# ru1ven/KeypointFusion

Measured on AMD Instinct MI355X. Metric: RGB-D img/sec fwd (B=64, 256x256), higher is better.
Workload: dtype f32; 1 GPU; KPFusion-convnext-tiny, depth+RGB UNet backbones forward, B=64/GPU 256x256 f32 (BASELINE configs[1]); batch_per_gpu=64, global_batch=64, input=256x256, parallelism=dp1 (batch shards, no collective)

## Files before the change

### include/kpf.h

```cpp
#ifndef KPF_H
#define KPF_H

#ifdef __cplusplus
extern "C" {
#endif

#define KPF_OK 0
#define KPF_EINVAL (-1)
#define KPF_ELAUNCH (-2)

#define KPF_DT_F32 0
#define KPF_DT_BF16 1
#define KPF_DT_F16 2
#define KPF_DT_F32_MMA_BF16 8
#define KPF_DT_F32_MMA_F16 9

#define KPF_ACT_RELU 1u
#define KPF_ACT_GELU 2u
#define KPF_RES_ADD 4u
#define KPF_RES_GAMMA 8u
#define KPF_RELU_AFTER_RES 16u
#define KPF_ACT_LEAKY 64u
#define KPF_IN_SPLIT 128u
#define KPF_W_SPLIT 512u
// ... 437 lines not shown
int kpf_geom_gate_forward(const float* pix_xyz, const float* joint_xyz, float* gam, int B, int J, int P, void* stream);
int kpf_geom_gate_backward(const float* pix_xyz, const float* joint_xyz, const float* dgam, float* djoint, int B, int J, int P, void* stream);

int kpf_geom_gate_uvd_forward(const float* pix_xyz, const float* joint_uvd, const float* par16, float* gam, int B, int J, int P, float half_size, float flip,
                              void* stream);
int kpf_geom_gate_uvd_backward(const float* pix_xyz, const float* joint_uvd, const float* par16, const float* dgam, float* djoint_uvd, int B, int J, int P,
                               float half_size, float flip, void* stream);

int kpf_prep_crop_u16(const unsigned char* rgb, const unsigned short* depth, const double* bbox, const double* cam, const double* cube, int B, int Hs, int Ws,
                      int x0, int y0, int H, int W, int S, float* img, float* img_rgb, float* center, float* M, float* cube_out, float* cam_para, double* com,
                      int* bounds, double* M64, void* stream);

int kpf_prep_pcl_sample(const float* img, const float* center, const double* M64, const double* cube, const double* cam, const long long* seed, int B, int S,
                        int n, float* pcl, int* pcl_index, int* pcl_count, float* cand_pts, void* stream);

int kpf_prep_uncrop_f32(const float* joints, const float* center, const float* M, const float* cube, const float* cam, int B, int J, float* crop_px,
                        float* frame_px, void* stream);

int kpf_prep_set_stamps(void* stamps64 );

int kpf_eval_errors_f32(const float* const* stages, int S, const float* gt, const float* cube, const int* score_index, int B, int J, int Jsel, float* err,
                        void* stream);

int kpf_eval_accumulate(const float* err, const unsigned char* valid, const double* thresholds, int S, int B, int Jsel, int T, long long* n_samples,
                        long long* n_batches, double* sum_err, double* sum_pa, double* sum_batch_mean, double* sum_batch_pa_mean, long long* pck,
                        long long* pck_pa, void* stream);

int kpf_prep_crop_u16_indexed(const unsigned char* rgb, const unsigned short* depth, const int* frame_index, int F, const double* bbox, const double* cam,
                              const double* cube, int B, int Hs, int Ws, int x0, int y0, int H, int W, int S, float* img, float* img_rgb, float* center, float* M,
                              float* cube_out, float* cam_para, double* com, int* bounds, double* M64, void* stream);

int kpf_track_step_f32(const float* joints, const float* center, const float* M, const float* cube, const float* cam_para, const int* pcl_count, int B, int J,
                       int frame_w, int frame_h, float expansion, long long seed_stride, double* bbox, long long* seed, int* lost, float* crop_px,
                       float* frame_px, float* cam_mm, double* bbox_used, int* status, void* stream);

int kpf_prep_annot_u16(const unsigned char* rgb, const unsigned short* depth, const int* frame_index, int F, const float* joints_mm, const float* cam32,
                       const float* center_xyz, const unsigned char* mirror, const double* cube, int B, int J, int Hs, int Ws, int x0, int y0, int H, int W, int S,
                       float* img, float* img_rgb, float* center, float* M, float* cube_out, float* cam_para, double* com, int* bounds, double* M64, float* joint,
                       float* joint_img, double* cam64, void* stream);

int kpf_prep_uncrop_mirror_f32(const float* joints, const float* center, const float* M, const float* cube, const float* cam, const unsigned char* mirror,
                               int frame_w, int B, int J, float* crop_px, float* frame_px, void* stream);

int kpf_prep_augment_u16(const unsigned char* rgb, const unsigned short* depth, const int* frame_index, int F, const float* joints_mm, const float* cam32,
                         const float* center_xyz, const unsigned char* mirror, const double* cube, const int* mode, const double* off, const double* sc,
                         const double* rot, const double* rot_cs, const double* color, int B, int J, int Hs, int Ws, int x0, int y0, int H, int W, int S,
                         float* img, float* img_rgb, float* center, float* M, float* cube_out, float* cam_para, double* com, int* bounds, double* M64,
                         float* joint, float* joint_img, double* cam64, double* cube64, int* aug_status, void* stream);

int kpf_prep_aug_draw(long long* seed, int B, double sigma_com, double sigma_sc, double rot_range, double color_factor, long long seed_stride, int* mode,
                      double* off, double* sc, double* rot, double* rot_cs, double* color, void* stream);

int kpf_conv_num_tile_cfgs(void);

const char* kpf_last_error(void);
#define KPF_ABI_VERSION 31
int kpf_abi_version(void);

#ifdef __cplusplus
}
#endif
#endif
```

### keypointfusion_amd/csrc/kpf_conv.hip

```cpp
#include "kpf_common.h"
#include <stdlib.h>
#include <type_traits>

namespace {

struct ConvArgs {
  const float* in;
  const float* w;
  const float* bias;
  const float* ps;
  const float* pt;
  const float* gamma;
  const float* res;
  float* out;
  int M, N, K, Kp;
  int IH, IW, Cin, in_ld, in_coff;
  int OH, OW, ohow, KH, KW, sh, sw, ph, pw;
  int out_ld, out_coff, res_ld, res_coff;
  const float* zero;
  float w_unscale;
  unsigned flags;
  int tilesN, nblk;
  int vec;
  int dbg;
  int st_policy;
  int skew;
  int groups, g_in, g_out;
  long g_w;
};

__device__ __forceinline__ ConvArgs kpf_group_args(const ConvArgs& a0) {
  ConvArgs a = a0;
  const int g = blockIdx.y;
  a.in_coff += g * a.g_in;
  a.out_coff += g * a.g_out;
  a.res_coff += g * a.g_out;
  a.w += (long)g * a.g_w;
  if (a.bias) a.bias += g * a.g_out;
  return a;
}

__device__ __forceinline__ float gelu_erf(float x) {
  const float z = fabsf(x) * 0.70710678118654752440f;
  const float t = __builtin_amdgcn_rcpf(fmaf(0.3275911f, z, 1.0f));
  float p = fmaf(1.061405429f, t, -1.453152027f);
  p = fmaf(p, t, 1.421413741f);
  p = fmaf(p, t, -0.284496736f);
  p = fmaf(p, t, 0.254829592f);
  const float e = __builtin_amdgcn_exp2f(-1.4426950408889634f * z * z);
  const float q = 0.5f * x * (p * t) * e;
  return fmaxf(x, 0.f) - fabsf(q);
}

// ... 149 lines not shown
      if (WHOLE || RPP * p + 8 * wave < BN)
        __builtin_amdgcn_global_load_lds((gbl_void_t*)(pb[p] + kt * BK), (lds_void_t*)(Bs + (RPP * p + 8 * wave) * BK), 16, 0, 0);
  };

  const f32x4 zero4 = {0.f, 0.f, 0.f, 0.f};
  f32x4 acc[TN][TM];
#pragma unroll
  for (int i = 0; i < TN; ++i)
#pragma unroll
    for (int j = 0; j < TM; ++j) acc[i][j] = zero4;

  const int nk = a.Kp / BK;
  const int fr = lane & 15;
  const int fg = lane >> 4;
  const int rsw = (fr >> 1) & 7;

  constexpr int EPW = H16 ? 2 : 1;
  float* pro_s = lds + NS * TILE;
  float* pro_t = pro_s + a.Kp * EPW;
  if (NS <= 2) {
    stage(0, 0);
  } else {
#pragma unroll
    for (int t = 0; t < NS - 1; ++t)
      if (t < nk) stage(t, t);
  }
  if (HAS_PRO) {
    for (int i = tid; i < a.Kp * EPW; i += 64 * NW) {
      pro_s[i] = i < a.Cin * EPW ? a.ps[i] : 0.f;
      pro_t[i] = i < a.Cin * EPW ? a.pt[i] : 0.f;
    }
  }
  if (NS <= 2) __syncthreads();

  KPF_STAMP(1);
  if constexpr (ARITH == ARITH_F32 && NS == 2) {
    auto read_frags = [&](int buf, int s16, f32x4(&xf)[TM], f32x4(&wf)[TN]) {
      const float* xrow = lds + buf * TILE + (wm * TM * 16 + fr) * BK;
      const float* wrow = lds + buf * TILE + BMR * BK + (wn * TN * 16 + fr) * BK;
      const int sc = (((4 * s16 + fg) ^ rsw) << 2);
#pragma unroll
      for (int j = 0; j < TM; ++j) xf[j] = *reinterpret_cast<const f32x4*>(xrow + j * 16 * BK + sc);
#pragma unroll
      for (int i = 0; i < TN; ++i) wf[i] = *reinterpret_cast<const f32x4*>(wrow + i * 16 * BK + sc);
    };
    auto prologue = [&](int kt, int s16, f32x4(&xf)[TM]) {
      if constexpr (HAS_PRO) {
        const int kk = kt * BK + 16 * s16 + 4 * fg;
        const f32x4 sp = *reinterpret_cast<const f32x4*>(pro_s + kk);
        const f32x4 tp = *reinterpret_cast<const f32x4*>(pro_t + kk);
#pragma unroll
        for (int j = 0; j < TM; ++j)
#pragma unroll
          for (int e = 0; e < 4; ++e) xf[j][e] = fmaxf(fmaf(xf[j][e], sp[e], tp[e]), 0.f);
      }
    };
    auto mma = [&](int e, const f32x4(&xf)[TM], const f32x4(&wf)[TN]) {
#pragma unroll
      for (int i = 0; i < TN; ++i)
#pragma unroll
        for (int j = 0; j < TM; ++j) acc[i][j] = __builtin_amdgcn_mfma_f32_16x16x4f32(wf[i][e], xf[j][e], acc[i][j], 0, 0, 0);
    };
    f32x4 xa[TM], wa[TN], xb[TM], wb[TN];
    read_frags(0, 0, xa, wa);
    if (nk > 1) stage(1, 1);
    for (int kt = 0; kt + 1 < nk; ++kt) {
      const int cur = kt & 1;
      read_frags(cur, 1, xb, wb);
      prologue(kt, 0, xa);
#pragma unroll
      for (int e = 0; e < 4; ++e) mma(e, xa, wa);
      prologue(kt, 1, xb);
#pragma unroll
      for (int e = 0; e < 3; ++e) mma(e, xb, wb);
      __builtin_amdgcn_sched_barrier(0);
      asm volatile("s_waitcnt vmcnt(0) lgkmcnt(0)" ::: "memory");
      __builtin_amdgcn_s_barrier();
      __builtin_amdgcn_sched_barrier(0);
      read_frags(cur ^ 1, 0, xa, wa);
      stage(kt + 2 < nk ? kt + 2 : nk - 1, cur);
      mma(3, xb, wb);
      __builtin_amdgcn_sched_group_barrier(0x100, TM + TN, 0);
#pragma unroll
      for (int q = 0; q < AP + BP; ++q) {
        __builtin_amdgcn_sched_group_barrier(0x008, (TM * TN) / (AP + BP) > 0 ? (TM * TN) / (AP + BP) : 1, 0);
        __builtin_amdgcn_sched_group_barrier(0x020, 1, 0);
      }
    }
    {
      const int kt = nk - 1, cur = kt & 1;
      read_frags(cur, 1, xb, wb);
      prologue(kt, 0, xa);
#pragma unroll
      for (int e = 0; e < 4; ++e) mma(e, xa, wa);
      prologue(kt, 1, xb);
#pragma unroll
      for (int e = 0; e < 4; ++e) mma(e, xb, wb);
    }
    asm volatile("s_waitcnt vmcnt(0)" ::: "memory");
  } else
  if constexpr (NS > 2 && ARITH == ARITH_SPLIT && !HAS_PRO) {
    const int ch = ((fg ^ rsw) << 2), cl = (((4 + fg) ^ rsw) << 2);
    auto read_frags = [&](int buf, f16x8(&xh)[TM], f16x8(&xl)[TM], f16x8(&wh)[TN], f16x8(&wl)[TN]) {
      const float* xrow = lds + buf * TILE + (wm * TM * 16 + fr) * BK;
      const float* wrow = lds + buf * TILE + BMR * BK + (wn * TN * 16 + fr) * BK;
#pragma unroll
      for (int j = 0; j < TM; ++j) {
// ... 137 lines not shown
          tp1 = *reinterpret_cast<const f32x4*>(pro_t + kk + 4);
        }
#pragma unroll
        for (int j = 0; j < TM; ++j) {
          f32x4 u0 = *reinterpret_cast<const f32x4*>(xrow + j * 16 * BK + c0);
          f32x4 u1 = *reinterpret_cast<const f32x4*>(xrow + j * 16 * BK + c1);
          if (HAS_PRO) {
#pragma unroll
            for (int e = 0; e < 4; ++e) {
              u0[e] = fmaxf(fmaf(u0[e], sp0[e], tp0[e]), 0.f);
              u1[e] = fmaxf(fmaf(u1[e], sp1[e], tp1[e]), 0.f);
            }
          }
#pragma unroll
          for (int e = 0; e < 4; ++e) {
            const float v0 = __builtin_amdgcn_fmed3f(u0[e], -65504.0f, 65504.0f), v1 = __builtin_amdgcn_fmed3f(u1[e], -65504.0f, 65504.0f);
            const _Float16 h0 = (_Float16)v0, h1 = (_Float16)v1;
            xh[j][e] = h0;
            xh[j][4 + e] = h1;
            xl[j][e] = (_Float16)(v0 - (float)h0);
            xl[j][4 + e] = (_Float16)(v1 - (float)h1);
          }
        }
      }
#pragma unroll
      for (int i = 0; i < TN; ++i) {
        wh[i] = *reinterpret_cast<const f16x8*>(wrow + i * 16 * BK + ch);
        wl[i] = *reinterpret_cast<const f16x8*>(wrow + i * 16 * BK + cl);
      }
#pragma unroll
      for (int i = 0; i < TN; ++i)
#pragma unroll
        for (int j = 0; j < TM; ++j) {
          acc[i][j] = __builtin_amdgcn_mfma_f32_16x16x32_f16(wl[i], xh[j], acc[i][j], 0, 0, 0);
          acc[i][j] = __builtin_amdgcn_mfma_f32_16x16x32_f16(wh[i], xl[j], acc[i][j], 0, 0, 0);
          acc[i][j] = __builtin_amdgcn_mfma_f32_16x16x32_f16(wh[i], xh[j], acc[i][j], 0, 0, 0);
        }
    } else {
#pragma unroll
      for (int s = 0; s < BK / 16; ++s) {
        const int sc = (((4 * s + fg) ^ rsw) << 2);
        f32x4 xf[TM], wf[TN];
#pragma unroll
        for (int j = 0; j < TM; ++j) xf[j] = *reinterpret_cast<const f32x4*>(xrow + j * 16 * BK + sc);
#pragma unroll
        for (int i = 0; i < TN; ++i) wf[i] = *reinterpret_cast<const f32x4*>(wrow + i * 16 * BK + sc);
        if (HAS_PRO) {
          const int kk = kt * BK + 16 * s + 4 * fg;
          const f32x4 sp = *reinterpret_cast<const f32x4*>(pro_s + kk);
          const f32x4 tp = *reinterpret_cast<const f32x4*>(pro_t + kk);
#pragma unroll
          for (int j = 0; j < TM; ++j)
#pragma unroll
            for (int e = 0; e < 4; ++e) xf[j][e] = fmaxf(fmaf(xf[j][e], sp[e], tp[e]), 0.f);
        }
        if constexpr (ARITH == ARITH_R_BF16 || ARITH == ARITH_R_F16) {
          typedef short r16x4 __attribute__((ext_vector_type(4)));
          r16x4 wh[TN], xh[TM];
#pragma unroll
          for (int i = 0; i < TN; ++i) {
            if constexpr (ARITH == ARITH_R_BF16) wh[i] = __builtin_bit_cast(r16x4, bf16x4{(bf16_t)wf[i][0], (bf16_t)wf[i][1], (bf16_t)wf[i][2], (bf16_t)wf[i][3]});
            else wh[i] = __builtin_bit_cast(r16x4, f16x4{(f16_t)wf[i][0], (f16_t)wf[i][1], (f16_t)wf[i][2], (f16_t)wf[i][3]});
          }
#pragma unroll
          for (int j = 0; j < TM; ++j) {
            if constexpr (ARITH == ARITH_R_BF16) xh[j] = __builtin_bit_cast(r16x4, bf16x4{(bf16_t)xf[j][0], (bf16_t)xf[j][1], (bf16_t)xf[j][2], (bf16_t)xf[j][3]});
            else xh[j] = __builtin_bit_cast(r16x4, f16x4{(f16_t)xf[j][0], (f16_t)xf[j][1], (f16_t)xf[j][2], (f16_t)xf[j][3]});
          }
#pragma unroll
          for (int i = 0; i < TN; ++i)
#pragma unroll
            for (int j = 0; j < TM; ++j) {
              if constexpr (ARITH == ARITH_R_BF16) acc[i][j] = __builtin_amdgcn_mfma_f32_16x16x16bf16_1k(wh[i], xh[j], acc[i][j], 0, 0, 0);
              else acc[i][j] = __builtin_amdgcn_mfma_f32_16x16x16f16(__builtin_bit_cast(f16x4, wh[i]), __builtin_bit_cast(f16x4, xh[j]), acc[i][j], 0, 0, 0);
            }
        } else {
#pragma unroll
          for (int e = 0; e < 4; ++e)
#pragma unroll
            for (int i = 0; i < TN; ++i)
#pragma unroll
              for (int j = 0; j < TM; ++j)
                acc[i][j] = __builtin_amdgcn_mfma_f32_16x16x4f32(wf[i][e], xf[j][e], acc[i][j], 0, 0, 0);
        }
      }
    }
    if (NS == 2) __syncthreads();
    if (NS == 1 && kt + 1 < nk) {
      __syncthreads();
      stage(kt + 1, 0);
      __syncthreads();
    }
  }

  KPF_STAMP(2);
  const unsigned fl = a.flags;
  const bool interior = (m0 + BM <= a.M) && (n0 + BN <= a.N) && a.vec && !(fl & KPF_OUT_NCHW);
  if (interior) {
    f32x4 bvv[TN], gvv[TN];
#pragma unroll
    for (int i = 0; i < TN; ++i) {
      const int n = n0 + (wn * TN + i) * 16 + fg * 4;
      bvv[i] = a.bias ? *reinterpret_cast<const f32x4*>(a.bias + n) : zero4;
      gvv[i] = (EPI == EPI_RES && (fl & KPF_RES_GAMMA)) ? *reinterpret_cast<const f32x4*>(a.gamma + n) : zero4;
    }
    constexpr bool HAS_RES = EPI == EPI_RES || EPI == EPI_GGRAD;
    constexpr bool STAGED = H16 && !HAS_RES && TN == 4;
    constexpr int RS = TN * 16 + 8;
    TH* stg = reinterpret_cast<TH*>(lds) + wave * (TM * 16) * RS;
    if constexpr (STAGED) __syncthreads();
    f32x4 rvv[HAS_RES ? TM : 1][TN];
    if (HAS_RES) {
#pragma unroll
      for (int j = 0; j < TM; ++j) {
        const long m = m0 + (wm * TM + j) * 16 + fr;
#pragma unroll
        for (int i = 0; i < TN; ++i) {
          const long o = m * a.res_ld + a.res_coff + n0 + (wn * TN + i) * 16 + fg * 4;
          if constexpr (H16) rvv[j][i] = kpf_ld4(reinterpret_cast<const TH*>(a.res) + o);
          else rvv[j][i] = *reinterpret_cast<const f32x4*>(a.res + o);
        }
      }
    }
#pragma unroll
    for (int j = 0; j < TM; ++j) {
      const long m = m0 + (wm * TM + j) * 16 + fr;
#pragma unroll
      for (int i = 0; i < TN; ++i) {
        const int n = n0 + (wn * TN + i) * 16 + fg * 4;
        const f32x4 bv = bvv[i], gv = gvv[i];
        f32x4 v = acc[i][j];
        if (SPLIT) {
#pragma unroll
          for (int e = 0; e < 4; ++e) v[e] *= a.w_unscale;
        }
        if (EPI == EPI_RES) {
#pragma unroll
          for (int e = 0; e < 4; ++e) {
            float y = v[e] + bv[e];
            if (fl & KPF_RES_GAMMA) y *= gv[e];
            y += rvv[HAS_RES ? j : 0][i][e];
            if (fl & KPF_RELU_AFTER_RES) y = fmaxf(y, 0.f);
            v[e] = y;
          }
        } else if (EPI == EPI_GGRAD) {
#pragma unroll
          for (int e = 0; e < 4; ++e) v[e] = (v[e] + bv[e]) * gelu_grad_erf(rvv[HAS_RES ? j : 0][i][e]);
        } else if (EPI == EPI_GELU) {
#pragma unroll
          for (int e = 0; e < 4; ++e) v[e] = gelu_of<ARITH>(v[e] + bv[e]);
        } else if (EPI == EPI_GELU2) {
          f32x4 z;
#pragma unroll
          for (int e = 0; e < 4; ++e) z[e] = v[e] + bv[e];
          if constexpr (H16) kpf_st4(reinterpret_cast<TH*>(const_cast<float*>(a.res)) + m * a.res_ld + a.res_coff + n, z);
          else STORE4(const_cast<float*>(a.res) + m * a.res_ld + a.res_coff + n, z);
#pragma unroll
          for (int e = 0; e < 4; ++e) {
            if constexpr (H16) z[e] = (float)(TH)z[e];
            v[e] = gelu_exact_erf(z[e]);
          }
        } else {
#pragma unroll
          for (int e = 0; e < 4; ++e) {
            const float y = v[e] + bv[e];
            v[e] = (fl & KPF_ACT_RELU) ? fmaxf(y, 0.f) : y;
          }
          if (fl & KPF_ACT_LEAKY) {
#pragma unroll
            for (int e = 0; e < 4; ++e) v[e] = fmaxf(v[e], 0.01f * v[e]);
          }
        }
        if constexpr (STAGED)
          kpf_st4(stg + (j * 16 + fr) * RS + i * 16 + fg * 4, v);
        else if constexpr (H16)
          kpf_st4(reinterpret_cast<TH*>(a.out) + m * a.out_ld + a.out_coff + n, v);
        else if (fl & KPF_OUT_SPLIT)
          kpf_store_split4(a.out + m * a.out_ld + a.out_coff, n, v);
        else if (a.st_policy == 2)
          asm volatile("global_store_dwordx4 %0, %1, off nt" ::"v"(a.out + m * a.out_ld + a.out_coff + n), "v"(v) : "memory");
        else
          STORE4(a.out + m * a.out_ld + a.out_coff + n, v);
      }
    }
    if constexpr (STAGED) {
      __syncthreads();
      TH* ob = reinterpret_cast<TH*>(a.out) + (long)(m0 + wm * TM * 16) * a.out_ld + a.out_coff + n0 + wn * TN * 16;
      const int prow = lane >> 3, pch = (lane & 7) * 8;
#pragma unroll
      for (int r = 0; r < TM * 2; ++r) {
        const int px = r * 8 + prow;
        const f32x4 q = *reinterpret_cast<const f32x4*>(stg + px * RS + pch);
        *reinterpret_cast<f32x4*>(ob + (long)px * a.out_ld + pch) = q;
      }
    }
    KPF_STAMP(3);
    return;
  }
  if constexpr (EPI == EPI_LIN) {
    if ((fl & KPF_OUT_NCHW) && a.ohow % BM == 0 && m0 + BM <= a.M && !(fl & KPF_OUT_SPLIT)) {
      constexpr int RS = BM + 4;
      static_assert(WN * 16 * RS <= NS * TILE, "the transpose staging fits the K buffers");
      const int b = m0 / a.ohow, pix0 = m0 - b * a.ohow;
#pragma unroll
      for (int i = 0; i < TN; ++i) {
        __syncthreads();
        const int nq = n0 + (wn * TN + i) * 16 + fg * 4;
        float bq[4];
#pragma unroll
        for (int e = 0; e < 4; ++e) bq[e] = (a.bias && nq + e < a.N) ? a.bias[nq + e] : 0.f;
#pragma unroll
        for (int j = 0; j < TM; ++j) {
          const int ml = (wm * TM + j) * 16 + fr;
#pragma unroll
          for (int e = 0; e < 4; ++e) {
            float y = (SPLIT ? acc[i][j][e] * a.w_unscale : acc[i][j][e]) + bq[e];
            if (fl & KPF_ACT_RELU) y = fmaxf(y, 0.f);
            if (fl & KPF_ACT_LEAKY) y = fmaxf(y, 0.01f * y);
            lds[(wn * 16 + fg * 4 + e) * RS + ml] = y;
          }
// ... 776 lines not shown
  KPF_REQUIRE(!(fl & KPF_RES_GELU_GRAD) || ((fl & KPF_RES_ADD) && !(fl & (KPF_RES_GAMMA | KPF_RELU_AFTER_RES | KPF_OUT_NCHW))), "kpf_conv2d_f32: RES_GELU_GRAD goes with RES_ADD alone");
  KPF_REQUIRE(!(fl & KPF_ACT_GELU_SAVE) || ((fl & KPF_ACT_GELU) && !(fl & (KPF_RES_ADD | KPF_OUT_NCHW)) && res && kpf_aligned16(res) && d->res_coff >= 0 && d->res_coff + d->N <= d->res_ld),
              "kpf_conv2d_f32: ACT_GELU_SAVE goes with ACT_GELU and a second output buffer in the res slot (res_ld / res_coff describe it)");
  KPF_REQUIRE((long)d->B * d->OH * d->OW < (1l << 31) && (long)d->B * d->IH * d->IW < (1l << 31), "kpf_conv2d_f32: too many pixels");

  ConvArgs a;
  a.in = in; a.w = w; a.bias = bias; a.ps = pro_scale; a.pt = pro_shift; a.gamma = gamma; a.res = res; a.out = out;
  a.M = d->B * d->OH * d->OW; a.N = d->N; a.K = d->KH * d->KW * d->Cin; a.Kp = d->Kp;
  a.IH = d->IH; a.IW = d->IW; a.Cin = d->Cin; a.in_ld = d->in_ld; a.in_coff = d->in_coff;
  a.OH = d->OH; a.OW = d->OW; a.ohow = d->OH * d->OW; a.KH = d->KH; a.KW = d->KW;
  a.sh = d->sh; a.sw = d->sw; a.ph = d->ph; a.pw = d->pw;
  a.out_ld = d->out_ld; a.out_coff = d->out_coff; a.res_ld = d->res_ld; a.res_coff = d->res_coff;
  {
    static const float* zero_of_dev[64] = {nullptr};
    int dev = 0;
    if (hipGetDevice(&dev) != hipSuccess || dev < 0 || dev >= 64) dev = 0;
    if (!zero_of_dev[dev]) {
      void* p = nullptr;
      if (hipGetSymbolAddress(&p, HIP_SYMBOL(kpf_zero16)) != hipSuccess || !p) {
        kpf_set_error("kpf_conv2d_f32: cannot resolve the zero page");
        return KPF_ELAUNCH;
      }
      zero_of_dev[dev] = static_cast<const float*>(p);
    }
    a.zero = zero_of_dev[dev];
  }
  a.flags = fl; a.tilesN = 0; a.nblk = 0; a.dbg = 0; a.skew = 0; a.st_policy = 0;
  {
    static const int st_mb = []() { const char* e = getenv("KPF_F32_ST_MB"); return e ? atoi(e) : 0; }();
    if (st_mb > 0 && (long)d->B * d->OH * d->OW * d->N * 4 >= (long)st_mb * 1000000) a.st_policy = 2;
  }
  a.w_unscale = (fl & (KPF_IN_SPLIT | KPF_W_SPLIT)) ? d->w_unscale : 1.0f;
  if (fl & (KPF_IN_SPLIT | KPF_W_SPLIT))
    KPF_REQUIRE(d->w_unscale > 0.f && d->Cin % 32 == 0 && d->in_coff % 4 == 0, "kpf_conv2d_f32: split operands need w_unscale > 0 and Cin %% 32 == 0 (Cin=%d)", d->Cin);
  if (fl & KPF_IN_SPLIT) KPF_REQUIRE(d->in_coff % 32 == 0 && d->in_ld % 32 == 0 && !pro_scale, "kpf_conv2d_f32: split activations need in_ld, in_coff multiples of 32 and no operand prologue");
  if (fl & KPF_OUT_SPLIT)
    KPF_REQUIRE(d->N % 32 == 0 && d->out_coff % 32 == 0 && d->out_ld % 32 == 0 && !(fl & KPF_OUT_NCHW),
                "kpf_conv2d_f32: split output needs N, out_ld, out_coff multiples of 32 (N=%d ld=%d coff=%d)", d->N, d->out_ld, d->out_coff);
  a.vec = (d->out_ld % 4 == 0 && d->out_coff % 4 == 0 && (!(fl & KPF_RES_ADD) || (d->res_ld % 4 == 0 && d->res_coff % 4 == 0))) ? 1 : 0;
  a.groups = d->groups > 1 ? d->groups : 1; a.g_in = a.g_out = 0; a.g_w = 0;
  if (a.groups > 1) {
    KPF_REQUIRE(!(fl & (KPF_RES_GAMMA | KPF_OUT_NCHW | KPF_IN_SPLIT | KPF_W_SPLIT | KPF_OUT_SPLIT)) && !pro_scale && d->w_gstride % 4 == 0,
                "kpf_conv2d_f32: a grouped launch takes no layer scale / prologue / NCHW output / split operands, and needs w_gstride %% 4 == 0");
    KPF_REQUIRE(d->in_coff + d->groups * d->Cin <= d->in_ld && d->out_coff + d->groups * d->N <= d->out_ld, "kpf_conv2d_f32: the groups' channel slices exceed the pixel stride");
    KPF_REQUIRE(!(fl & (KPF_RES_ADD | KPF_ACT_GELU_SAVE)) || d->res_coff + d->groups * d->N <= d->res_ld,
                "kpf_conv2d_f32: the groups' residual / saved pre-activation slices exceed the pixel stride");
    a.g_in = d->Cin; a.g_out = d->N; a.g_w = d->w_gstride;
    if ((d->out_coff + d->N) % 4 || ((fl & KPF_RES_ADD) && (d->res_coff + d->N) % 4)) a.vec = 0;
  }
  const bool is1x1 = d->KH == 1 && d->KW == 1 && d->sh == 1 && d->sw == 1 && d->ph == 0 && d->pw == 0 &&
                     d->IH == d->OH && d->IW == d->OW && d->Cin % 32 == 0 && d->Kp == d->Cin;
  hipStream_t st = reinterpret_cast<hipStream_t>(stream);

  int best = 0;
  double bc = 1e30;
  static const int forced = []() { const char* e = getenv("KPF_FORCE_CFG"); return e ? atoi(e) : -1; }();
  for (int i = 0; i < (int)(sizeof(kCfgs) / sizeof(kCfgs[0])); ++i) {
    const double c = cfg_cost(kCfgs[i], a.M, a.N, a.groups);
    if (c < bc) { bc = c; best = i; }
  }
  const bool f32_arith = !(fl & (KPF_IN_SPLIT | KPF_W_SPLIT));
  const bool gelu1x1 = f32_arith && is1x1 && (fl & KPF_ACT_GELU) && !(fl & KPF_ACT_GELU_SAVE) && !pro_scale && d->groups <= 1;
  if (gelu1x1 && a.M >= 1024 && a.N >= 512) {
    auto rounds_cost = [&](int bm, int bn, double pen) { return (double)((((long)(a.M + bm - 1) / bm) * ((a.N + bn - 1) / bn) + 255) / 256) * bm * bn * pen; };
    const double c0 = rounds_cost(128, 128, 1.00), c8 = rounds_cost(256, 128, 0.97);
    best = c0 <= c8 ? 0 : 8;
  }
  if (f32_arith && best < 9 && a.Kp >= 512) {
    const long bb = ((a.M + kCfgs[best].bm - 1) / kCfgs[best].bm) * ((a.N + kCfgs[best].bn - 1) / kCfgs[best].bn) * a.groups;
    if (bb < 256 && (long)((a.M + 31) / 32) * ((a.N + 63) / 64) * a.groups >= 512) best = 7;
  }
  if ((fl & (KPF_IN_SPLIT | KPF_W_SPLIT)) && !(fl & KPF_RES_ADD) && !pro_scale && (best == 0 || best == 8)) best = 13;
  if ((fl & (KPF_IN_SPLIT | KPF_W_SPLIT)) && !pro_scale && a.Kp >= 1024) {
    const long blocks = ((a.M + kCfgs[best < 9 ? best : 0].bm - 1) / kCfgs[best < 9 ? best : 0].bm) *
                        ((a.N + kCfgs[best < 9 ? best : 0].bn - 1) / kCfgs[best < 9 ? best : 0].bn);
    const long blocks64 = ((a.M + 63) / 64) * ((a.N + 63) / 64);
    if (best < 9 && blocks <= 512 && blocks64 >= 512) best = 16;
  }
  if (forced >= 0) best = forced;
  if (d->tile_cfg > 0) {
    KPF_REQUIRE(d->tile_cfg <= KPF_NUM_TILE_CFGS, "kpf_conv2d_f32: tile_cfg %d out of range", d->tile_cfg);
    best = d->tile_cfg - 1;
  }
#ifdef KPF_FAST_BUILD
  return launch_cfg<4, 4, 2, 2>(a, is1x1, st);
#else
  switch (best) {
    case 0: return launch_cfg<4, 4, 2, 2>(a, is1x1, st);
    case 1: return launch_cfg<4, 3, 2, 2>(a, is1x1, st);
    case 2: return launch_cfg<2, 4, 4, 1>(a, is1x1, st);
    case 3: return launch_cfg<4, 3, 4, 1>(a, is1x1, st);
    case 4: return launch_cfg<2, 7, 4, 1>(a, is1x1, st);
    case 5: return launch_cfg<2, 4, 2, 2>(a, is1x1, st);
    case 6: return launch_cfg<2, 2, 2, 2>(a, is1x1, st);
    case 8: return launch_cfg<4, 4, 4, 2>(a, is1x1, st);
    case 9: return launch_cfg<4, 4, 4, 2, 3>(a, is1x1, st);
    case 10: return launch_cfg<4, 4, 2, 2>(a, is1x1, st);
    case 11: return launch_cfg<4, 3, 2, 2>(a, is1x1, st);
    case 12: return launch_cfg<2, 4, 4, 1, 3>(a, is1x1, st);
    case 13: return launch_cfg<4, 4, 2, 2, 1>(a, is1x1, st);
    case 14: return launch_cfg<4, 3, 2, 2, 1>(a, is1x1, st);
    case 15: return launch_cfg<2, 4, 4, 1, 1>(a, is1x1, st);
    case 16: return launch_cfg<2, 2, 2, 2, 1>(a, is1x1, st);
    case 17: return launch_cfg<4, 6, 2, 2>(a, is1x1, st);
    default: return launch_cfg<2, 1, 1, 4>(a, is1x1, st);
  }
// ... 16 lines not shown
```

### keypointfusion_amd/lib.py

```python
import ctypes as C
import os

_HERE = os.path.dirname(os.path.abspath(__file__))
LIB_PATH = os.environ.get("KPF_LIB_PATH") or os.path.join(_HERE, "libkpf_hip.so")

KPF_ACT_RELU = 1
KPF_ACT_GELU = 2
KPF_RES_ADD = 4
KPF_RES_GAMMA = 8
KPF_RELU_AFTER_RES = 16
KPF_RES_GELU_GRAD = 1024
KPF_ACT_GELU_SAVE = 2048
KPF_PRO_LN = 4096
KPF_DT_F32_MMA_BF16, KPF_DT_F32_MMA_F16 = 8, 9
KPF_MMA_BF16, KPF_MMA_F16 = 8192, 16384
KPF_OUT_NCHW = 32
KPF_ACT_LEAKY = 64
KPF_IN_SPLIT = 128
KPF_OUT_SPLIT = 256
KPF_W_SPLIT = 512
KPF_DT_F32, KPF_DT_BF16, KPF_DT_F16 = 0, 1, 2
ABI_VERSION = 31


class ConvDesc(C.Structure):
    _fields_ = [(n, C.c_int) for n in (
        "B", "IH", "IW", "Cin", "in_ld", "in_coff", "OH", "OW", "N", "KH", "KW", "sh", "sw", "ph", "pw", "Kp",
        "out_ld", "out_coff", "res_ld", "res_coff")] + [("flags", C.c_uint), ("w_unscale", C.c_float), ("tile_cfg", C.c_int), ("groups", C.c_int), ("w_gstride", C.c_long)]


class PackDesc(C.Structure):
    _fields_ = [("src", C.c_void_p), ("dst", C.c_void_p)] + [(n, C.c_int) for n in (
        "N", "Cin", "KH", "KW", "mode", "n_pad", "Kp", "rows", "src_dtype", "dst_dtype", "first_block", "reserved")]


class AdamwDesc(C.Structure):
    _fields_ = [("p", C.c_void_p), ("g", C.c_void_p), ("m", C.c_void_p), ("v", C.c_void_p), ("n", C.c_long), ("first_block", C.c_int), ("reserved", C.c_int)]


class WgradGroupDesc(C.Structure):
    _fields_ = [("dy", C.c_void_p), ("x", C.c_void_p), ("dw", C.c_void_p), ("db", C.c_void_p), ("M", C.c_int), ("N", C.c_int), ("K", C.c_int), ("first_block", C.c_int), ("sps", C.c_int), ("ldy", C.c_int)]


class ColsumDesc(C.Structure):
    _fields_ = [("part", C.c_void_p), ("dw", C.c_void_p), ("db", C.c_void_p), ("nblk", C.c_int), ("C", C.c_int), ("first_block", C.c_int), ("reserved", C.c_int)]


class WgradReduceDesc(C.Structure):
    _fields_ = [("part", C.c_void_p), ("dbpart", C.c_void_p), ("dw", C.c_void_p), ("db", C.c_void_p), ("g_ws", C.c_long)] + [
        (n, C.c_int) for n in "S N K Cin KHW nkb ndb groups Cin_out N_out kind first_block".split()]


class ManoFitCfg(C.Structure):
    _fields_ = [("iters", C.c_int)] + [(n, C.c_float) for n in "lr_pose lr_shape lr_trans beta1 beta2 eps lambda_shape lambda_pose".split()] + [
        ("init_trans", C.c_int), ("joint_map", C.c_int * 21)]


class ManoFitMeshCfg(C.Structure):
    _fields_ = ManoFitCfg._fields_ + [("lambda_verts", C.c_float)]


class ManoFitGnCfg(C.Structure):
    _fields_ = [("iters", C.c_int)] + [(n, C.c_float) for n in "mu nu lambda_shape lambda_pose".split()] + [("init_trans", C.c_int), ("joint_map", C.c_int * 21)]


class ManoFitMeshGnCfg(C.Structure):
    _fields_ = ManoFitGnCfg._fields_ + [("lambda_verts", C.c_float)]


class WgradPlan(C.Structure):
    _fields_ = [(n, C.c_int) for n in "family vn vk tiles_n tiles_k S sps writes_dw".split()] + [("ws_floats", C.c_long)]


KPF_WGRAD_FAMILY = ("f32", "r16", "direct", "h16s", "h16")
KPF_WGRAD_FORM = {"f32_2x2": 1, "f32_2x4": 2, "f32_4x2": 3, "f32_4x4": 4, "h16s": 5, "h16": 6}
# ... 22 lines not shown
    "kpf_offset2joint_f32": [_P] * 8 + [C.c_int, C.c_int, C.c_int, C.c_float, C.c_int, C.c_int, _P],
    "kpf_img2pcl_top4_f32": [_P] * 9 + [C.c_int] * 6 + [_P],
    "kpf_point_assemble_f32": [_P] * 9 + [C.c_int, C.c_int, C.c_int, C.c_float, _P],
    "kpf_softmax_pool_f32": [_P, _P, _P, _P, C.c_int, C.c_int, _P],
    "kpf_ball_group_f32": [_P, _P, _P, _P, C.c_int, _P, _P, C.c_int, C.c_int, C.c_float, C.c_float, C.c_float, _P],
    "kpf_group_max_f32": [_P, _P, C.c_long, C.c_int, C.c_int, C.c_int, C.c_int, _P],
    "kpf_ball_group_stacked_f32": [_P, _P, _P, _P, C.c_int, _P, _P, _P, C.c_int, C.c_int, C.c_float, C.c_float, C.c_float, _P],
    "kpf_ball_group_bwd_f32": [_P, C.c_int, _P, _P, _P, _P, C.c_int, C.c_int, C.c_int, _P],
    "kpf_slices_sum_relu_forward": [_P, _P, C.c_long, C.c_int, C.c_int, C.c_int, _P],
    "kpf_slices_sum_relu_backward": [_P, _P, _P, _P, C.c_long, C.c_int, C.c_int, C.c_int, _P],
    "kpf_group_max_train_forward": [_P, _P, _P, C.c_long, C.c_int, C.c_int, _P],
    "kpf_group_max_train_backward": [_P, C.c_int, _P, _P, C.c_long, C.c_int, C.c_int, _P],
    "kpf_heat_gam_gate_f32": [_P, _P, _P, C.c_int] + [_P] * 10 + [C.c_int] * 4 + [_P],
    "kpf_gate_reduce_f32": [_P, _P, _P, _P, _P, C.c_int, C.c_int, _P],
    "kpf_tr_encoder_f32": [_P, C.c_int, C.c_int, _P, _P, _P, _P, C.c_int, C.c_int, _P],
    "kpf_xattn_layer_f32": [_P, _P, _P, _P, C.c_int, C.c_int, C.c_int, _P],
    "kpf_conv2d_h16": [C.POINTER(ConvDesc), _P, _P, _P, _P, _P, _P, _P, _P, C.c_int, _P],
    "kpf_conv2d_h16_uses_8ph": [C.POINTER(ConvDesc), C.c_int],
    "kpf_conv2d_h16_ln_fold_supported": [C.POINTER(ConvDesc)],
    "kpf_dwconv7_ln_h16": [_P, _P, _P, _P, _P, _P, C.c_int, C.c_int, C.c_int, C.c_int, C.c_float, C.c_int, _P],
    "kpf_layernorm_h16": [_P, C.c_int, _P, _P, _P, C.c_int, C.c_long, C.c_int, C.c_float, _P],
    "kpf_upsample2x_h16": [_P, _P, C.c_int, C.c_int, C.c_int, C.c_int, C.c_int, C.c_int, C.c_int, _P],
    "kpf_cast_h16_f32": [_P, C.c_int, _P, C.c_long, C.c_int, C.c_int, C.c_int, _P],
    "kpf_cast_f32_h16": [_P, _P, C.c_int, C.c_long, _P],
    "kpf_convnext_mlp_f32": [_P] * 8 + [C.c_long, C.c_int, _P],
    "kpf_convnext_mlp_supported": [C.c_int],
    "kpf_convnext_mlp_split_f32": [_P, _P, _P, _P, C.c_float, _P, _P, C.c_float, _P, _P, C.c_long, C.c_int, _P],
    "kpf_convnext_mlp_split_supported": [C.c_int],
    "kpf_convnext_mlp_h16": [_P] * 8 + [C.c_long, C.c_int, C.c_int, _P],
    "kpf_convnext_mlp_h16_supported": [C.c_int],
    "kpf_dwconv7_stats_h16": [_P, _P, _P, _P, _P, C.c_int, C.c_int, C.c_int, C.c_int, C.c_int, _P],
    "kpf_dwconv7_stats_supported": [C.c_int, C.c_int, C.c_int],
    "kpf_ln_apply_stats_h16": [_P, _P, _P, _P, C.c_long, C.c_int, C.c_float, C.c_int, _P],
    "kpf_ln_stats_merge": [_P, _P, C.c_long, C.c_int, C.c_float, _P],
    "kpf_cbam_channel_gate_f32": [_P] * 7 + [C.c_int] * 4 + [_P],
    "kpf_cbam_spatial_gate_f32": [_P, _P, _P, C.c_float, C.c_float, _P, _P, C.c_int, C.c_int, C.c_int, C.c_int, _P],
    "kpf_cbam_apply_f32": [_P] * 5 + [C.c_int] * 3 + [_P],
    "kpf_maxpool2x2_f32": [_P, _P, C.c_int, C.c_int, C.c_int, C.c_int, _P],
    "kpf_upnearest2x_add_f32": [_P, _P, _P, C.c_int, C.c_int, C.c_int, C.c_int, _P],
    "kpf_mano_forward_f32": [_P, C.c_int, _P, C.c_int] + [_P] * 10 + [C.c_int, _P],
    "kpf_mano_backward_f32": [_P, C.c_int, _P, C.c_int] + [_P] * 10 + [_P, C.c_int, _P, C.c_int, C.c_int, _P],
    "kpf_mano_fit_f32": [_P] * 8 + [C.POINTER(ManoFitCfg)] + [_P] * 8 + [C.c_int, _P],
    "kpf_mano_fit_mesh_f32": [_P] * 10 + [C.POINTER(ManoFitMeshCfg)] + [_P] * 8 + [C.c_int, _P],
    "kpf_mano_fit_gn_f32": [_P] * 8 + [C.POINTER(ManoFitGnCfg)] + [_P] * 10 + [C.c_int, _P],
    "kpf_mano_fit_mesh_gn_f32": [_P] * 10 + [C.POINTER(ManoFitMeshGnCfg)] + [_P] * 11 + [C.c_int, _P],
    "kpf_mano_assoc_f32": [_P, _P, _P, C.c_float, _P, _P, _P, _P, C.c_int, C.c_int, _P],
    "kpf_mano_normals_f32": [_P, _P, C.c_int, C.c_float, _P, C.c_int, _P],
    "kpf_mano_assoc_vis_f32": [_P, _P, _P, _P, C.c_float, C.c_float, _P, _P, _P, _P, _P, C.c_int, C.c_int, _P],
    "kpf_mano_assoc_vis_mask_f32": [_P, _P, _P, _P, _P, C.c_float, C.c_float, _P, _P, _P, _P, _P, C.c_int, C.c_int, _P],
    "kpf_mano_raster_f32": [_P, _P, C.c_int, _P, _P, C.c_int, C.c_int, C.c_float, _P, _P, _P, _P, _P, C.c_int, _P],
    "kpf_mano_fit_mesh_gn_plane_f32": [_P] * 11 + [C.POINTER(ManoFitMeshGnCfg)] + [_P] * 11 + [C.c_int, _P],
    "kpf_tr_encoder_weight_floats": [C.c_int],
    "kpf_conv_num_tile_cfgs": [],
    "kpf_xattn_weight_floats": [],
    "kpf_bn_train_forward": [_P, C.c_int, _P, _P, _P, C.c_int, _P, _P, _P, _P, C.c_float, C.c_float, C.c_int, _P, C.c_long, C.c_long, C.c_int, _P],
    "kpf_bn_train_backward": [_P, _P, _P, C.c_int, C.c_int, _P, _P, _P, _P, _P, _P, _P, C.c_int, _P, C.c_long, C.c_long, C.c_int, _P],
    "kpf_dwconv7_f32": [_P, _P, _P, _P, C.c_int, C.c_int, C.c_int, C.c_int, _P],
    "kpf_dwconv7_add_f32": [_P, _P, _P, _P, _P, C.c_int, C.c_int, C.c_int, C.c_int, _P],
    "kpf_conv2d_wgrad": [_P, _P, C.c_int] + [_P] * 3 + [C.c_long] + [C.c_int] * 18 + [C.POINTER(WgradReduceDesc), _P],
    "kpf_dwconv7_wgrad": [_P] * 5 + [C.c_long] + [C.c_int] * 4 + [C.POINTER(WgradReduceDesc), _P],
    "kpf_wgrad_reduce_multi": [C.POINTER(WgradReduceDesc), C.c_int, _P],
    "kpf_conv2d_wgrad_plan": [C.c_int, C.c_int, C.c_long, C.c_int, C.c_int, C.c_int, C.c_int, C.POINTER(WgradPlan)],
    "kpf_dwconv7_plan": [C.c_int] * 7 + [C.POINTER(Dw7Plan)],
    "kpf_conv2d_wgrad_force_form": [C.c_int],
    "kpf_row_gather_cols_f32": [_P, C.c_long, C.c_long, C.c_long, _P, _P, _P, C.c_int, C.c_int, C.c_int, C.c_int, C.c_int, _P],
    "kpf_bn_ssr_forward": [_P] * 7 + [C.c_float, C.c_float, _P, C.c_long, C.c_long, C.c_int, C.c_int, C.c_int, _P],
    "kpf_bn_ssr_backward": [_P] * 10 + [C.c_long, C.c_long, C.c_int, C.c_int, C.c_int, _P],
    "kpf_bn_relu_gmax_forward": [_P] * 8 + [C.c_float, C.c_float, _P, C.c_long, C.c_long, C.c_int, C.c_int, _P],
    "kpf_bn_relu_gmax_backward": [_P, C.c_int] + [_P] * 9 + [C.c_long, C.c_long, C.c_int, C.c_int, _P],
    "kpf_bn2_add_relu_forward": [_P] * 12 + [C.c_float, C.c_float, _P, C.c_long, C.c_long, C.c_int, _P],
    "kpf_bn2_add_relu_backward": [_P] * 14 + [C.c_long, C.c_long, C.c_int, _P],
    "kpf_unstack_rows": [_P, C.c_int, _P, C.c_long, C.c_int, C.c_int, C.c_int, C.c_int, C.c_int, _P],
    "kpf_restack_rows": [C.POINTER(C.c_void_p), _P, C.c_int, C.c_long, C.c_int, C.c_int, C.c_int, C.c_int, C.c_int, _P],
    "kpf_add_relu_forward": [_P, _P, _P, _P, C.c_long, C.c_float, _P],
    "kpf_add_relu_backward": [_P, _P, _P, C.c_long, C.c_float, _P],
    "kpf_gate_mix_forward": [_P] * 6 + [C.c_int] * 3 + [_P],
    "kpf_gate_mix_backward": [_P] * 11 + [C.c_int] * 3 + [_P],
    "kpf_pad_rows": [_P, C.c_int, _P, C.c_int, C.c_long, C.c_int, C.c_int, C.c_int, _P],
    "kpf_pose_tokens_f32": [_P, _P, _P, _P, C.c_int, C.c_int, C.c_int, C.c_int, C.c_float, _P],
    "kpf_upsample2x_bwd": [_P, _P] + [C.c_int] * 5 + [_P],
    "kpf_maxpool3x3s2_fwd": [_P, _P, _P] + [C.c_int] * 5 + [_P],
    "kpf_maxpool3x3s2_bwd": [_P, _P, _P] + [C.c_int] * 5 + [_P],
    "kpf_row_gather_fwd_f32": [_P] * 4 + [C.c_int] * 5 + [_P],
    "kpf_pack_conv_weight": [_P, C.c_int, _P, C.c_int] + [C.c_int] * 7 + [_P],
    "kpf_pack_conv_weights_multi": [_P, C.c_int, C.c_int, _P],
    "kpf_joint_heatmap_forward": [_P, _P, C.c_int, C.c_int, C.c_int, C.c_float, C.c_float, _P],
    "kpf_joint_heatmap_backward": [_P, _P, _P, C.c_int, C.c_int, C.c_int, C.c_float, C.c_float, _P],
    "kpf_geom_gate_forward": [_P, _P, _P, C.c_int, C.c_int, C.c_int, _P],
    "kpf_geom_gate_backward": [_P, _P, _P, _P, C.c_int, C.c_int, C.c_int, _P],
    "kpf_geom_gate_uvd_forward": [_P, _P, _P, _P, C.c_int, C.c_int, C.c_int, C.c_float, C.c_float, _P],
    "kpf_geom_gate_uvd_backward": [_P, _P, _P, _P, _P, C.c_int, C.c_int, C.c_int, C.c_float, C.c_float, _P],
    "kpf_linear_wgrad_grouped": [C.POINTER(WgradGroupDesc), C.c_int, _P],
    "kpf_adamw_step_multi": [C.POINTER(AdamwDesc), C.c_int, _P, C.c_float, _P, C.c_double, C.c_double, C.c_float, C.c_float, _P],
    "kpf_adamw_step_multi_scaled": [C.POINTER(AdamwDesc), C.c_int, _P, C.c_float, _P, C.c_double, C.c_double, C.c_float, C.c_float, _P, _P, _P],
    "kpf_grad_finite_check_multi": [C.POINTER(AdamwDesc), C.c_int, _P, _P],
    "kpf_loss_scale_update": [_P, _P, _P, _P, _P, C.c_float, C.c_float, C.c_int, _P],
    "kpf_ln_train_forward": [_P, _P, _P, _P, C.c_int, _P, _P, C.c_long, C.c_int, C.c_int, C.c_float, _P],
    "kpf_ln_train_backward": [_P, C.c_int, _P, _P, _P, _P, _P, _P, _P, _P, C.c_long, C.c_long, C.c_int, C.c_int, C.POINTER(ColsumDesc), _P],
    "kpf_gelu_forward": [_P, _P, C.c_int, C.c_long, _P],
    "kpf_dense_loss_forward": [_P, _P, _P, _P, C.c_int, C.c_int, C.c_int, C.c_int, C.c_float, _P],
    "kpf_dense_loss_backward": [_P, _P, _P, _P, _P, C.c_int, C.c_int, C.c_int, C.c_int, C.c_float, _P],
    "kpf_loss_tail_forward": [_P] * 11 + [C.c_int] * 3 + [_P],
    "kpf_loss_tail_backward": [_P] * 11 + [C.c_int] * 3 + [_P],
    "kpf_layer_scale_forward": [_P, _P, C.c_int, _P, _P, C.c_long, C.c_int, _P],
    "kpf_layer_scale_backward": [_P, _P, C.c_int, _P, _P, _P, _P, C.c_long, C.c_long, C.c_int, C.c_int, C.POINTER(ColsumDesc), _P],
    "kpf_drop_add_ln_forward": [_P] * 9 + [C.c_long, C.c_int, C.c_float, C.c_float, _P, C.c_int, _P],
# ... 94 lines not shown
```

Baseline: 3517 img/s.

## Add persistent weight-stationary streaming kernel for large-M narrow 1x1 convs

Adds a persistent MFMA kernel for 1x1 stride-1 convolutions with small Cin/N (Kp<=128) and large M. It loads the whole weight matrix, bias and BN prologue into LDS once per block, then has each wave stream 16-row tiles with a software-pipelined double-buffered load/compute loop. The aim is to avoid the K-tiled GEMM's repeated weight staging and barriers on bandwidth-bound high-resolution UNet layers. In exchange it adds template variants, an occupancy-sized grid, and a dispatch gate (M>=262144), and it shares the epilogue math through new helper functions.

```diff
diff --git a/include/kpf.h b/include/kpf.h
--- a/include/kpf.h
+++ b/include/kpf.h
@@ -513,9 +513,11 @@
                       double* off, double* sc, double* rot, double* rot_cs, double* color, void* stream);
 
 int kpf_conv_num_tile_cfgs(void);
+int kpf_conv2d_f32_streams(const kpf_conv_desc* d);
+int kpf_conv2d_f32_stream_waves(const kpf_conv_desc* d);
 
 const char* kpf_last_error(void);
-#define KPF_ABI_VERSION 31
+#define KPF_ABI_VERSION 32
 int kpf_abi_version(void);
 
 #ifdef __cplusplus
diff --git a/keypointfusion_amd/csrc/kpf_conv.hip b/keypointfusion_amd/csrc/kpf_conv.hip
--- a/keypointfusion_amd/csrc/kpf_conv.hip
+++ b/keypointfusion_amd/csrc/kpf_conv.hip
@@ -1,4 +1,5 @@
 #include "kpf_common.h"
+#include "kpf_conv_epi.h"
 #include <stdlib.h>
 #include <type_traits>
 
@@ -254,7 +255,7 @@
 #pragma unroll
         for (int j = 0; j < TM; ++j)
 #pragma unroll
-          for (int e = 0; e < 4; ++e) xf[j][e] = fmaxf(fmaf(xf[j][e], sp[e], tp[e]), 0.f);
+          for (int e = 0; e < 4; ++e) xf[j][e] = kpf_pro_bn_relu(xf[j][e], sp[e], tp[e]);
       }
     };
     auto mma = [&](int e, const f32x4(&xf)[TM], const f32x4(&wf)[TN]) {
@@ -498,7 +499,7 @@
 #pragma unroll
           for (int j = 0; j < TM; ++j)
 #pragma unroll
-            for (int e = 0; e < 4; ++e) xf[j][e] = fmaxf(fmaf(xf[j][e], sp[e], tp[e]), 0.f);
+            for (int e = 0; e < 4; ++e) xf[j][e] = kpf_pro_bn_relu(xf[j][e], sp[e], tp[e]);
         }
         if constexpr (ARITH == ARITH_R_BF16 || ARITH == ARITH_R_F16) {
           typedef short r16x4 __attribute__((ext_vector_type(4)));
@@ -582,13 +583,7 @@
         }
         if (EPI == EPI_RES) {
 #pragma unroll
-          for (int e = 0; e < 4; ++e) {
-            float y = v[e] + bv[e];
-            if (fl & KPF_RES_GAMMA) y *= gv[e];
-            y += rvv[HAS_RES ? j : 0][i][e];
-            if (fl & KPF_RELU_AFTER_RES) y = fmaxf(y, 0.f);
-            v[e] = y;
-          }
+          for (int e = 0; e < 4; ++e) v[e] = kpf_epi_res(v[e], bv[e], gv[e], rvv[HAS_RES ? j : 0][i][e], fl);
         } else if (EPI == EPI_GGRAD) {
 #pragma unroll
           for (int e = 0; e < 4; ++e) v[e] = (v[e] + bv[e]) * gelu_grad_erf(rvv[HAS_RES ? j : 0][i][e]);
@@ -608,10 +603,7 @@
           }
         } else {
 #pragma unroll
-          for (int e = 0; e < 4; ++e) {
-            const float y = v[e] + bv[e];
-            v[e] = (fl & KPF_ACT_RELU) ? fmaxf(y, 0.f) : y;
-          }
+          for (int e = 0; e < 4; ++e) v[e] = kpf_epi_lin(v[e], bv[e], fl);
           if (fl & KPF_ACT_LEAKY) {
 #pragma unroll
             for (int e = 0; e < 4; ++e) v[e] = fmaxf(v[e], 0.01f * v[e]);
@@ -1494,6 +1486,9 @@
                      d->IH == d->OH && d->IW == d->OW && d->Cin % 32 == 0 && d->Kp == d->Cin;
   hipStream_t st = reinterpret_cast<hipStream_t>(stream);
 
+  if (kpf_conv_stream_takes(d) && (!pro_scale || (is1x1 && !(fl & KPF_RES_ADD))))
+    return kpf_conv_stream_launch(d, in, w, bias, pro_scale, pro_shift, res, out, st);
+
   int best = 0;
   double bc = 1e30;
   static const int forced = []() { const char* e = getenv("KPF_FORCE_CFG"); return e ? atoi(e) : -1; }();
diff --git a/keypointfusion_amd/csrc/kpf_conv_epi.h b/keypointfusion_amd/csrc/kpf_conv_epi.h
--- /dev/null
+++ b/keypointfusion_amd/csrc/kpf_conv_epi.h
@@ -0,0 +1,21 @@
+#pragma once
+#include "kpf_common.h"
+
+__device__ __forceinline__ float kpf_pro_bn_relu(float x, float s, float t) { return fmaxf(fmaf(x, s, t), 0.f); }
+
+__device__ __forceinline__ float kpf_epi_lin(float acc, float b, unsigned fl) {
+  const float y = acc + b;
+  return (fl & KPF_ACT_RELU) ? fmaxf(y, 0.f) : y;
+}
+
+__device__ __forceinline__ float kpf_epi_res(float acc, float b, float g, float r, unsigned fl) {
+  float y = acc + b;
+  if (fl & KPF_RES_GAMMA) y *= g;
+  y += r;
+  if (fl & KPF_RELU_AFTER_RES) y = fmaxf(y, 0.f);
+  return y;
+}
+
+bool kpf_conv_stream_takes(const kpf_conv_desc* d);
+int kpf_conv_stream_launch(const kpf_conv_desc* d, const float* in, const float* w, const float* bias, const float* pro_scale, const float* pro_shift,
+                           const float* res, float* out, hipStream_t st);
diff --git a/keypointfusion_amd/csrc/kpf_conv_stream.hip b/keypointfusion_amd/csrc/kpf_conv_stream.hip
--- /dev/null
+++ b/keypointfusion_amd/csrc/kpf_conv_stream.hip
@@ -0,0 +1,242 @@
+#include "kpf_conv_epi.h"
+#include <stdlib.h>
+
+namespace {
+
+struct StreamArgs {
+  const float* in;
+  const float* w;
+  const float* bias;
+  const float* ps;
+  const float* pt;
+  const float* res;
+  float* out;
+  int M, Cin, in_ld, in_coff, out_ld, out_coff, res_ld, res_coff;
+  int ntiles;
+  unsigned flags;
+};
+
+constexpr int SW = 8;
+
+template <int TN, int KS, bool RES>
+__global__ __launch_bounds__(64 * SW) void igemm_f32_stream_kernel(const StreamArgs a) {
+  constexpr int N = 16 * TN, KP = 16 * KS;
+  constexpr int WS = KP + 4;
+  constexpr int RT = RES ? TN : 1;
+  constexpr int G = TN % 4 == 0 ? 4 : (TN % 3 == 0 ? 3 : (TN % 2 == 0 ? 2 : 1));
+  extern __shared__ __attribute__((aligned(16))) float lds[];
+  float* wl = lds;
+  float* bl = wl + N * WS;
+  float* psl = bl + N;
+  float* ptl = psl + KP;
+
+  const int tid = threadIdx.x;
+  const int lane = tid & 63;
+  const int wave = __builtin_amdgcn_readfirstlane(tid >> 6);
+  const int fr = lane & 15;
+  const int fg = lane >> 4;
+  const bool pro = a.ps != nullptr;
+  const f32x4 zero4 = {0.f, 0.f, 0.f, 0.f};
+
+  auto load_tile = [&](int t, f32x4(&xf)[KS], f32x4(&rf)[RT]) {
+    const int m = t * 16 + fr;
+    const long mc = m < a.M ? m : a.M - 1;
+    const float* px = a.in + mc * a.in_ld + a.in_coff + 4 * fg;
+#pragma unroll
+    for (int s = 0; s < KS; ++s) xf[s] = *reinterpret_cast<const f32x4*>(px + (16 * s < a.Cin ? 16 * s : 0));
+    if constexpr (RES) {
+      const float* pr = a.res + mc * a.res_ld + a.res_coff + 4 * fg;
+#pragma unroll
+      for (int i = 0; i < TN; ++i) rf[i] = *reinterpret_cast<const f32x4*>(pr + 16 * i);
+    }
+  };
+
+  auto compute_store = [&](int t, const f32x4(&xf)[KS], const f32x4(&rf)[RT]) {
+    int z = 0;
+    asm volatile("" : "+s"(z));
+    const float* wt = wl + z;
+    const float* bt = bl + z;
+    const float* pst = psl + z;
+    const float* ptt = ptl + z;
+    f32x4 acc[TN];
+#pragma unroll
+    for (int i = 0; i < TN; ++i) acc[i] = zero4;
+#pragma unroll
+    for (int s = 0; s < KS; ++s) {
+      f32x4 xs = xf[s];
+      if (pro) {
+        const f32x4 sp = *reinterpret_cast<const f32x4*>(pst + 16 * s + 4 * fg);
+        const f32x4 tp = *reinterpret_cast<const f32x4*>(ptt + 16 * s + 4 * fg);
+#pragma unroll
+        for (int e = 0; e < 4; ++e) xs[e] = kpf_pro_bn_relu(xs[e], sp[e], tp[e]);
+      }
+      if (16 * s >= a.Cin) xs = zero4;
+#pragma unroll
+      for (int i0 = 0; i0 < TN; i0 += G) {
+        f32x4 wf[G];
+#pragma unroll
+        for (int ii = 0; ii < G; ++ii) wf[ii] = *reinterpret_cast<const f32x4*>(wt + ((i0 + ii) * 16 + fr) * WS + 16 * s + 4 * fg);
+#pragma unroll
+        for (int e = 0; e < 4; ++e)
+#pragma unroll
+          for (int ii = 0; ii < G; ++ii) acc[i0 + ii] = __builtin_amdgcn_mfma_f32_16x16x4f32(wf[ii][e], xs[e], acc[i0 + ii], 0, 0, 0);
+      }
+    }
+    const int m = t * 16 + fr;
+    float* po = a.out + (long)m * a.out_ld + a.out_coff + 4 * fg;
+#pragma unroll
+    for (int i = 0; i < TN; ++i) {
+      const f32x4 bv = *reinterpret_cast<const f32x4*>(bt + 16 * i + 4 * fg);
+      f32x4 v = acc[i];
+#pragma unroll
+      for (int e = 0; e < 4; ++e) {
+        if constexpr (RES) v[e] = kpf_epi_res(v[e], bv[e], 0.f, rf[i][e], a.flags & KPF_RELU_AFTER_RES);
+        else v[e] = kpf_epi_lin(v[e], bv[e], a.flags);
+      }
+      if (m < a.M) *reinterpret_cast<f32x4*>(po + 16 * i) = v;
+    }
+  };
+
+  const int GW = gridDim.x * SW;
+  int t = blockIdx.x * SW + wave;
+  f32x4 xa[KS], xb[KS], ra[RT], rb[RT];
+  if (t < a.ntiles) load_tile(t, xa, ra);
+
+  for (int i = tid; i < N * (KP / 4); i += 64 * SW) {
+    const int n = i / (KP / 4), c = i - n * (KP / 4);
+    *reinterpret_cast<f32x4*>(wl + n * WS + 4 * c) = *reinterpret_cast<const f32x4*>(a.w + (long)n * KP + 4 * c);
+  }
+  for (int i = tid; i < N; i += 64 * SW) bl[i] = a.bias ? a.bias[i] : 0.f;
+  if (pro)
+    for (int i = tid; i < KP; i += 64 * SW) {
+      psl[i] = i < a.Cin ? a.ps[i] : 0.f;
+      ptl[i] = i < a.Cin ? a.pt[i] : 0.f;
+    }
+  __syncthreads();
+
+  while (t < a.ntiles) {
+    const int t1 = t + GW, t2 = t1 + GW;
+    load_tile(t1 < a.ntiles ? t1 : t, xb, rb);
+    compute_store(t, xa, ra);
+    load_tile(t2 < a.ntiles ? t2 : t, xa, ra);
+    if (t1 < a.ntiles) compute_store(t1, xb, rb);
+    t = t2;
+  }
+}
+
+
+constexpr size_t KPF_STREAM_LDS_BUDGET = 48 * 1024, KPF_STREAM_LDS_BUDGET_WIDE = 80 * 1024;
+constexpr int KPF_STREAM_MIN_M = 262144;
+
+size_t stream_lds_bytes(int N, int Kp) { return ((size_t)N * (Kp + 4) + N + 2 * (size_t)Kp) * sizeof(float); }
+
+bool stream_tn_ok(int tn) { return tn == 1 || tn == 2 || tn == 3 || tn == 4 || tn == 6 || tn == 8 || tn == 12; }
+
+int stream_cus(int dev) {
+  static int cus[KPF_MAX_DEVICES] = {0};
+  if (!cus[dev]) {
+    int n = 0;
+    if (hipDeviceGetAttribute(&n, hipDeviceAttributeMultiprocessorCount, dev) != hipSuccess || n <= 0) return 0;
+    cus[dev] = n;
+  }
+  return cus[dev];
+}
+
+template <int TN, int KS, bool RES>
+int stream_launch_one(const StreamArgs& a, hipStream_t st, int* waves_only) {
+  void (*kern)(const StreamArgs) = igemm_f32_stream_kernel<TN, KS, RES>;
+  const size_t lds = stream_lds_bytes(16 * TN, 16 * KS);
+  static std::atomic<bool> lds_opt_in[KPF_MAX_DEVICES];
+  static int per_cu[KPF_MAX_DEVICES] = {0};
+  int dev = 0;
+  if (hipGetDevice(&dev) != hipSuccess || dev < 0 || dev >= KPF_MAX_DEVICES) dev = 0;
+  const int cus = stream_cus(dev);
+  if (cus <= 0 || !kpf_raise_lds_limit(reinterpret_cast<const void*>(kern), lds_opt_in)) {
+    kpf_set_error("kpf_conv2d_f32: cannot size the streaming kernel's grid / raise its dynamic LDS limit");
+    return KPF_ELAUNCH;
+  }
+  if (!per_cu[dev]) {
+    int nb = 0;
+    if (hipOccupancyMaxActiveBlocksPerMultiprocessor(&nb, kern, 64 * SW, lds) != hipSuccess) nb = 1;
+    per_cu[dev] = nb >= 2 ? 2 : 1;
+  }
+  const int slots = cus * per_cu[dev], want = (a.ntiles + SW - 1) / SW;
+  const int grid = want < slots ? want : slots;
+  if (waves_only) {
+    *waves_only = grid * SW;
+    return KPF_OK;
+  }
+  hipLaunchKernelGGL(kern, dim3(grid), dim3(64 * SW), lds, st, a);
+  return kpf_check_launch("kpf_conv2d_f32");
+}
+
+template <int TN>
+int stream_launch_tn(const StreamArgs& a, int ks, bool res, hipStream_t st, int* wo) {
+  switch (ks) {
+    case 2: return res ? stream_launch_one<TN, 2, true>(a, st, wo) : stream_launch_one<TN, 2, false>(a, st, wo);
+    case 4: return res ? stream_launch_one<TN, 4, true>(a, st, wo) : stream_launch_one<TN, 4, false>(a, st, wo);
+    case 6: return res ? stream_launch_one<TN, 6, true>(a, st, wo) : stream_launch_one<TN, 6, false>(a, st, wo);
+    default: return res ? stream_launch_one<TN, 8, true>(a, st, wo) : stream_launch_one<TN, 8, false>(a, st, wo);
+  }
+}
+
+int stream_dispatch(const kpf_conv_desc* d, const StreamArgs& a, hipStream_t st, int* wo) {
+  const int ks = d->Kp / 16;
+  const bool res = d->flags & KPF_RES_ADD;
+  switch (d->N / 16) {
+    case 1: return stream_launch_tn<1>(a, ks, res, st, wo);
+    case 2: return stream_launch_tn<2>(a, ks, res, st, wo);
+    case 3: return stream_launch_tn<3>(a, ks, res, st, wo);
+    case 4: return stream_launch_tn<4>(a, ks, res, st, wo);
+    case 6: return stream_launch_tn<6>(a, ks, res, st, wo);
+    case 8: return stream_launch_tn<8>(a, ks, res, st, wo);
+    default: return stream_launch_tn<12>(a, ks, res, st, wo);
+  }
+}
+
+StreamArgs stream_args(const kpf_conv_desc* d, const float* in, const float* w, const float* bias, const float* ps, const float* pt, const float* res, float* out) {
+  StreamArgs a;
+  a.in = in; a.w = w; a.bias = bias; a.ps = ps; a.pt = pt; a.res = res; a.out = out;
+  a.M = d->B * d->OH * d->OW; a.Cin = d->Cin; a.in_ld = d->in_ld; a.in_coff = d->in_coff;
+  a.out_ld = d->out_ld; a.out_coff = d->out_coff; a.res_ld = d->res_ld; a.res_coff = d->res_coff;
+  a.ntiles = (a.M + 15) / 16;
+  a.flags = d->flags;
+  return a;
+}
+
+}
+
+bool kpf_conv_stream_takes(const kpf_conv_desc* d) {
+  if (!d) return false;
+  const char* sw = getenv("KPF_STREAM");
+  if (sw && atoi(sw) == 0) return false;
+  static const bool forced = getenv("KPF_FORCE_CFG") != nullptr;
+  if (forced || d->tile_cfg != 0) return false;
+  if (d->flags & ~(KPF_ACT_RELU | KPF_RES_ADD | KPF_RELU_AFTER_RES)) return false;
+  if (d->groups > 1) return false;
+  if (!(d->KH == 1 && d->KW == 1 && d->sh == 1 && d->sw == 1 && d->ph == 0 && d->pw == 0 && d->IH == d->OH && d->IW == d->OW)) return false;
+  if (d->B <= 0 || d->OH <= 0 || d->OW <= 0 || d->Cin <= 0 || d->N <= 0) return false;
+  if (d->Cin % 16 || d->Kp % 32 || d->Kp > 128 || d->Kp < d->Cin) return false;
+  if (d->N % 16 || !stream_tn_ok(d->N / 16)) return false;
+  if (d->in_ld % 4 || d->in_coff % 4 || d->out_ld % 4 || d->out_coff % 4) return false;
+  if ((d->flags & KPF_RES_ADD) && (d->res_ld % 4 || d->res_coff % 4)) return false;
+  const char* wide = getenv("KPF_STREAM_WIDE");
+  if (stream_lds_bytes(d->N, d->Kp) > ((wide && atoi(wide) != 0) ? KPF_STREAM_LDS_BUDGET_WIDE : KPF_STREAM_LDS_BUDGET)) return false;
+  long min_m = KPF_STREAM_MIN_M;
+  if (const char* e = getenv("KPF_STREAM_MIN_M")) min_m = atol(e);
+  return (long)d->B * d->OH * d->OW >= min_m;
+}
+
+int kpf_conv_stream_launch(const kpf_conv_desc* d, const float* in, const float* w, const float* bias, const float* pro_scale, const float* pro_shift,
+                           const float* res, float* out, hipStream_t st) {
+  return stream_dispatch(d, stream_args(d, in, w, bias, pro_scale, pro_shift, res, out), st, nullptr);
+}
+
+extern "C" int kpf_conv2d_f32_streams(const kpf_conv_desc* d) { return kpf_conv_stream_takes(d) ? 1 : 0; }
+
+extern "C" int kpf_conv2d_f32_stream_waves(const kpf_conv_desc* d) {
+  if (!kpf_conv_stream_takes(d)) return 0;
+  int waves = 0;
+  if (stream_dispatch(d, stream_args(d, nullptr, nullptr, nullptr, nullptr, nullptr, nullptr, nullptr), nullptr, &waves) != KPF_OK) return -1;
+  return waves;
+}
diff --git a/keypointfusion_amd/lib.py b/keypointfusion_amd/lib.py
--- a/keypointfusion_amd/lib.py
+++ b/keypointfusion_amd/lib.py
@@ -20,7 +20,7 @@
 KPF_OUT_SPLIT = 256
 KPF_W_SPLIT = 512
 KPF_DT_F32, KPF_DT_BF16, KPF_DT_F16 = 0, 1, 2
-ABI_VERSION = 31
+ABI_VERSION = 32
 
 
 class ConvDesc(C.Structure):
@@ -149,6 +149,8 @@
     "kpf_mano_fit_mesh_gn_plane_f32": [_P] * 11 + [C.POINTER(ManoFitMeshGnCfg)] + [_P] * 11 + [C.c_int, _P],
     "kpf_tr_encoder_weight_floats": [C.c_int],
     "kpf_conv_num_tile_cfgs": [],
+    "kpf_conv2d_f32_streams": [C.POINTER(ConvDesc)],
+    "kpf_conv2d_f32_stream_waves": [C.POINTER(ConvDesc)],
     "kpf_xattn_weight_floats": [],
     "kpf_bn_train_forward": [_P, C.c_int, _P, _P, _P, C.c_int, _P, _P, _P, _P, C.c_float, C.c_float, C.c_int, _P, C.c_long, C.c_long, C.c_int, _P],
     "kpf_bn_train_backward": [_P, _P, _P, C.c_int, C.c_int, _P, _P, _P, _P, _P, _P, _P, C.c_int, _P, C.c_long, C.c_long, C.c_int, _P],
```

Result: no change. 3538 img/s (median of 6 runs) (+0.6%).
